# haoningwu3639/StoryGen

Measured on AMD Instinct MI355X. Metric: UNet denoising steps/sec @512x512, 3 prior-frame ctx, bs=1, higher is better.
Workload: dtype f16; 1 GPU; BASELINE configs[1]: StoryGen denoising loop, 512x512 (64x64x4 latent), R=3 prior frames, CFG batch 3, DDIM, SD-1.5 UNet + attn3 (909M params, synthetic fp16 weights); stage=multi-image-condition, samples_per_gpu=1, parallelism=dp1 (one sample per GPU, final all-gather), hipgraph=True, dedup_identical_reference_samples=True, overlap_ref_pass_of_next_step=True, ref_ahead=1, warmup_run=5, split_graphs=False, stream_priority=False, ref_pass_on_cus=0, ref_pass_eager=False, paired_gemm_launches=True, paired_text_image_attention=False, groupnorm_stats_from_epilogues=True, fp16_block_stream=False

## Files before the change

### include/storygen_hip.h

```cpp
#ifndef STORYGEN_HIP_H
#define STORYGEN_HIP_H

#include <stddef.h>
#include <stdint.h>

#ifdef __cplusplus
extern "C" {
#endif

#define SG_OK        0
#define SG_EINVAL   (-1)
#define SG_EUNSUP   (-2)
#define SG_ELAUNCH  (-3)
#define SG_EARCH    (-4)

typedef void* sg_stream_t;
typedef uint16_t sg_half;

int          sg_version(void);
const char*  sg_last_error(void);
int          sg_device_arch(void);
int          sg_device_cus(void);

#define SG_EPI_LINEAR 0
// ... 80 lines not shown
    sg_half*       y;  int64_t ldy;
    int32_t        M, C;
    float          eps;
    int32_t        hidden_split;
} sg_ff_desc;

size_t sg_ff_fused_pack_bytes(int32_t C);
int sg_ff_geglu_fused_f16(const sg_ff_desc* d, sg_stream_t stream);

typedef struct sg_attn_desc {
    const sg_half* q;  int64_t ldq, bsq;
    const sg_half* k;  int64_t ldk, bsk;
    const sg_half* vt; int64_t ldvt, bsvt;
    sg_half*       o;  int64_t ldo, bso;
    int32_t B, H, Nq, Nk, D;
    int32_t kv_batches;
    float   scale;
    const sg_half* k2;  int64_t bsk2;
    const sg_half* vt2; int64_t bsvt2;
    int32_t Nk2, kv2_batches;
} sg_attn_desc;

int sg_attn_fwd_f16(const sg_attn_desc* d, sg_stream_t stream);

int sg_attn_fwd_pair_f16(const sg_attn_desc* d0, const sg_attn_desc* d1, sg_stream_t stream);

enum {
    SG_ATTN_D40_LOOP    = 0,
    SG_ATTN_SHARED_BODY = 1,
    SG_ATTN_GENERAL     = 2,
    SG_ATTN_LEAN        = 3,
    SG_ATTN_KSPLIT      = 4,
    SG_ATTN_LSE         = 5,
    SG_ATTN_F8          = 6
};
typedef struct sg_attn_plan {
    int32_t family, waves, stages, workgroups;
} sg_attn_plan;
typedef struct sg_attn_pair_plan {
    int32_t shared, first;
    sg_attn_plan p0, p1;
    int32_t workgroups;
} sg_attn_pair_plan;
int sg_attn_fwd_plan(const sg_attn_desc* d, int32_t lse, sg_attn_plan* out);
int sg_attn_fwd_pair_plan(const sg_attn_desc* d0, const sg_attn_desc* d1, sg_attn_pair_plan* out);

typedef struct sg_groupnorm_desc {
    const void*    x;  int64_t ldx;
    int32_t        x_f32;
    int32_t        y_pad_w;
    sg_half*       y;  int64_t ldy;
    sg_half*       xcopy; int64_t ldxc;
    const sg_half* gamma; const sg_half* beta;
    int32_t B, HW, C, groups;
    float   eps;
    int32_t silu;
    void*   workspace; size_t workspace_bytes;
    const float* pstats[2];
    int32_t pstats_rows[2], pstats_c0[2], pstats_nc[2];
    const float*   split_ws; int32_t split_count;
    const sg_half* split_bias;
    const float*   split_rowbias; int64_t split_rowbias_ld;
    const void*    split_res; int64_t split_ldr; int32_t split_res_f32;
    void*          split_out; int64_t split_ldo; int32_t split_out_f32;
    int32_t        split_round_f16;
} sg_groupnorm_desc;

// ... 184 lines not shown
```

### storygen_amd/csrc/attention.hip

```cpp
#include "attention_kernel.h"
#include <float.h>

using namespace sgattn;


static int attn_params(const sg_attn_desc* d, AttnParams& p, const char* who) {
    SG_REQUIRE(d != nullptr, "%s: null descriptor", who);
    SG_REQUIRE(d->q && d->k && d->vt && d->o, "%s: null q/k/vt/o", who);
    SG_REQUIRE(d->B > 0 && d->H > 0 && d->Nq > 0 && d->Nk > 0, "%s: bad shape", who);
    if (d->D != 40 && d->D != 80 && d->D != 160)
        return sg_set_error(SG_EUNSUP, "%s: head dim %d not in {40, 80, 160}", who, d->D);
    SG_REQUIRE(d->Nq <= (1 << 30) && d->Nk <= (1 << 30), "%s: Nq and Nk must not exceed 2^30", who);
    SG_REQUIRE(d->scale > 0.f && d->scale <= FLT_MAX, "%s: scale must be finite and > 0", who);
    SG_REQUIRE(d->kv_batches >= 0 && d->kv_batches <= d->B, "%s: kv_batches must be in [0, B]", who);
    SG_REQUIRE(d->kv_batches == 0 || 2 * (int64_t)d->kv_batches >= d->B, "%s: kv_batches must be 0 or at least B / 2", who);
    SG_REQUIRE(d->ldq % 8 == 0 && d->ldk % 8 == 0 && d->ldvt % 8 == 0 && d->ldo % 4 == 0, "%s: row strides", who);
    SG_REQUIRE(d->bsq % 8 == 0 && d->bsk % 8 == 0 && d->bsvt % 8 == 0 && d->bso % 4 == 0, "%s: batch strides", who);
    SG_REQUIRE(sg_aligned16(d->q) && sg_aligned16(d->k) && sg_aligned16(d->vt) && sg_aligned16(d->o), "%s: 16-byte alignment", who);
    const int64_t hd = (int64_t)d->H * d->D;
    SG_REQUIRE(d->ldq >= hd && d->ldk >= hd && d->ldo >= hd, "%s: token stride smaller than H*D", who);
    SG_REQUIRE(d->ldvt >= ((d->Nk + 7) & ~7), "%s: ldvt must cover Nk rounded up to 8 keys", who);
    SG_REQUIRE((int64_t)d->D * d->ldvt < (1ll << 31), "%s: VT head slab too large for 32-bit offsets", who);
    SG_REQUIRE(d->ldk < (1ll << 25), "%s: K tile (64 ldk) too large for 32-bit offsets", who);
    p = AttnParams{};
    p.q = reinterpret_cast<const f16*>(d->q); p.ldq = d->ldq; p.bsq = d->bsq;
    p.k = reinterpret_cast<const f16*>(d->k); p.ldk = d->ldk; p.bsk = d->bsk;
    p.vt = reinterpret_cast<const f16*>(d->vt); p.ldvt = d->ldvt; p.bsvt = d->bsvt;
    p.o = reinterpret_cast<f16*>(d->o); p.ldo = d->ldo; p.bso = d->bso;
    p.B = d->B; p.H = d->H; p.Nq = d->Nq; p.Nk = d->Nk;
    p.kv_batches = d->kv_batches > 0 ? d->kv_batches : d->B;
    p.scale_log2 = d->scale * 1.44269504088896340736f;
    if (d->kv2_batches > 0) {
        SG_REQUIRE(d->k2 && d->vt2 && d->Nk2 > 0 && d->kv2_batches <= p.kv_batches, "%s: kv2_batches needs k2, vt2, Nk2 and at most kv_batches rows", who);
        SG_REQUIRE(d->bsk2 % 8 == 0 && d->bsvt2 % 8 == 0 && sg_aligned16(d->k2) && sg_aligned16(d->vt2), "%s: k2 / vt2 strides and alignment", who);
        SG_REQUIRE(d->ldvt >= ((d->Nk2 + 7) & ~7), "%s: ldvt must cover Nk2 rounded up to 8 keys", who);
        p.k2 = reinterpret_cast<const f16*>(d->k2); p.bsk2 = d->bsk2;
        p.vt2 = reinterpret_cast<const f16*>(d->vt2); p.bsvt2 = d->bsvt2;
        p.Nk2 = d->Nk2; p.kv2 = d->kv2_batches;
    }
    return SG_OK;
}


static bool attn_big(const sg_attn_desc* d) { return (long)sg_cdiv(d->Nq, 128) * d->H * d->B >= 512; }

static int attn_plan_grid(sg_attn_plan& pl, const sg_attn_desc* d, int family, int waves, int stages, const char* who) {
    const int64_t wgs = (int64_t)sg_cdiv(d->Nq, family == SG_ATTN_KSPLIT ? 32 : 32 * waves) * d->H * d->B;
    SG_REQUIRE(wgs < (1ll << 31), "%s: %lld workgroups do not fit a grid", who, (long long)wgs);
    pl.family = family; pl.waves = waves; pl.stages = stages; pl.workgroups = (int32_t)wgs;
    return SG_OK;
}

static int attn_plan(const sg_attn_desc* d, bool lse, sg_attn_plan& pl, const char* who) {
    if (lse) return attn_plan_grid(pl, d, SG_ATTN_LSE, 4, 3, who);
    const bool big = attn_big(d);
    const SgOptions& opt = sg_options();
    if (d->D == 40) {
        if (big && opt.attn_d40_general) return attn_plan_grid(pl, d, SG_ATTN_GENERAL, 4, 3, who);
        if (big && opt.attn_lean) return attn_plan_grid(pl, d, SG_ATTN_LEAN, 4, 3, who);
        return attn_plan_grid(pl, d, opt.attn_d40_loop == 1 ? SG_ATTN_SHARED_BODY : SG_ATTN_D40_LOOP, big ? 4 : 2, big ? 3 : 2, who);
    }
    if (d->D == 160 && opt.attn_d160 == 4 && d->Nq <= 256 && d->Nk > KVBLK && (long)sg_cdiv(d->Nq, 32) * d->H * d->B <= 256)
        return attn_plan_grid(pl, d, SG_ATTN_KSPLIT, 4, 1, who);
    return attn_plan_grid(pl, d, SG_ATTN_GENERAL, 4, 3, who);
}

static int attn_launch(const AttnParams& p, int D, const sg_attn_plan& pl, hipStream_t st) {
    const bool big = pl.waves == 4;
    switch (pl.family) {
    case SG_ATTN_LSE:
        if (D == 40) launch_attn<40, 4, 3, true, false, true>(p, st);
        else if (D == 80) launch_attn<80, 4, 3, true>(p, st);
        else launch_attn<160, 4, 3, true>(p, st);
        return SG_OK;
    case SG_ATTN_D40_LOOP: big ? launch_attn_d40<4, 3>(p, st) : launch_attn_d40<2, 2>(p, st); return SG_OK;
    case SG_ATTN_SHARED_BODY: big ? launch_attn<40, 4, 3>(p, st) : launch_attn<40, 2, 2>(p, st); return SG_OK;
    case SG_ATTN_LEAN: launch_attn<40, 4, 3, false, true>(p, st); return SG_OK;
    case SG_ATTN_KSPLIT: launch_attn_ksplit<160, 4>(p, st); return SG_OK;
    case SG_ATTN_GENERAL:
        if (D == 40) launch_attn<40, 4, 3, false, false, true>(p, st);
        else if (D == 80) launch_attn<80, 4, 3>(p, st);
        else launch_attn<160, 4, 3>(p, st);
        return SG_OK;
    }
    return sg_set_error(SG_EINVAL, "attention: internal: no kernel for plan family %d", pl.family);
}

static int attn_fwd(const sg_attn_desc* d, float* lse2, sg_stream_t stream) {
    const char* who = lse2 ? "sg_attn_fwd_lse_f16" : "sg_attn_fwd_f16";
    AttnParams p;
    sg_attn_plan pl;
    if (int rc = attn_params(d, p, "sg_attn_fwd_f16")) return rc;
    if (int rc = attn_plan(d, lse2 != nullptr, pl, "sg_attn_fwd_f16")) return rc;
    p.lse2 = lse2;
    if (int rc = attn_launch(p, d->D, pl, (hipStream_t)stream)) return rc;
    SG_CHECK_LAUNCH(who);
    return SG_OK;
}

extern "C" int sg_attn_fwd_f16(const sg_attn_desc* d, sg_stream_t stream) { return attn_fwd(d, nullptr, stream); }

extern "C" int sg_attn_fwd_plan(const sg_attn_desc* d, int32_t lse, sg_attn_plan* out) {
    SG_REQUIRE(out != nullptr, "sg_attn_fwd_plan: null plan");
    AttnParams p;
    if (int rc = attn_params(d, p, "sg_attn_fwd_plan")) return rc;
    return attn_plan(d, lse != 0, *out, "sg_attn_fwd_plan");
}

static int attn_pair_plan(const sg_attn_desc* d0, const sg_attn_desc* d1, sg_attn_pair_plan& pr, const char* who) {
    const SgOptions& opt = sg_options();
    const bool same = d0->D == d1->D && d0->B == d1->B && d0->H == d1->H && d0->Nq == d1->Nq;
// ... 55 lines not shown
```

### storygen_amd/csrc/attention_kernel.h

```cpp
#pragma once
#include "common.h"
#include <stdlib.h>
#include <type_traits>

namespace sgattn {


constexpr int KVBLK = 64;
constexpr float RESCALE_THR = 6.0f;

struct AttnParams {
    const f16* q; long ldq, bsq;
    const f16* k; long ldk, bsk;
    const f16* vt; long ldvt, bsvt;
    f16* o; long ldo, bso;
    int B, H, Nq, Nk, kv_batches, nqb;
    const f16* k2; long bsk2; const f16* vt2; long bsvt2; int Nk2, kv2;
    float scale_log2;
    float* lse2;
};

__device__ __forceinline__ void glds16(const f16* g, char* lds_wave_base) {
    __builtin_amdgcn_global_load_lds((const __attribute__((address_space(1))) void*)g,
                                     (__attribute__((address_space(3))) void*)lds_wave_base, 16, 0, 0);
}
template <int N>
__device__ __forceinline__ void wait_vmcnt() {
    asm volatile("s_waitcnt vmcnt(%0)" ::"n"(N) : "memory");
}

template <int D>
__device__ __forceinline__ int kswz(int row) {
    return D == 40 ? 0 : (D == 80 ? ((row >> 3) & 1) : ((row >> 2) & 3));
}

constexpr int F40_KPAD = 2688;
constexpr int F40_ONES = 128;

template <int D, int NIMG>
constexpr int attn_smem_bytes() {
    return D == 40 ? F40_KPAD + NIMG * (KVBLK * D * 2 + D * 128 + F40_ONES) : NIMG * (KVBLK * D * 2 + D * 128) + (D % 16 == 0 ? 0 : 16);
}

template <int D, int NW, int S, bool LSE, bool LEAN = false, bool GENERAL = false, bool KSPLIT = false>
__device__ __forceinline__ void attn_fwd_body(const AttnParams& p, char* smem, const int block, const int nblocks) {
    constexpr int SUB = KSPLIT ? NW : 1;
    constexpr bool F40 = D == 40 && !GENERAL;
    constexpr int DC = D / 8;
    constexpr int NDK = (D + 15) / 16;
    constexpr int DT = (D + 31) / 32;
    constexpr int KROW = D * 2;
    constexpr int K_BYTES = KVBLK * KROW;
    constexpr int V_BYTES = D * 128;
    constexpr int K_SEG = K_BYTES / 1024, V_SEG = V_BYTES / 1024, NSEG = K_SEG + V_SEG;
    constexpr int TSTAGE = K_BYTES + V_BYTES + (F40 ? F40_ONES : 0);
    constexpr int STAGE = SUB * TSTAGE;
    constexpr int RING0 = F40 ? F40_KPAD : 0;
    constexpr int MAXL = (NSEG + NW - 1) / NW;
    constexpr int REM = NSEG % NW;
    static_assert(KSPLIT ? (S == 1 && !LSE && !(D == 40 && !GENERAL)) : (S == 2 || S == 3), "2 or 3 stages; key split: one stage of NW tiles");
    static_assert(!KSPLIT || NW * (8 + DT * 64) * 64 <= S * SUB * (KVBLK * D * 2 + D * 128), "the merge images of the waves fit the dead ring");
    static_assert((S - 1) * MAXL < 64, "vmcnt is a 6-bit counter");
    static_assert(RING0 + S * STAGE + (F40 || D % 16 == 0 ? 0 : 16) <= attn_smem_bytes<D, S * SUB>(), "LDS size");
    static_assert(!F40 || (32 * KROW + 16 <= F40_KPAD && F40_KPAD % 128 == 0), "K pad constants of both 32-key blocks");

    const int t = threadIdx.x, lane = t & 63, l31 = lane & 31, hi = lane >> 5;
    const int wave = __builtin_amdgcn_readfirstlane(t >> 6);
    const int work = xcd_remap(block, nblocks);
    const int bh = work / p.nqb, qb = work - bh * p.nqb;
    const int h = bh / p.B, b = bh - h * p.B;
    const int kvb = b < p.kv_batches ? b : b - (p.B - p.kv_batches);
    const bool short_row = kvb < p.kv2;
    const int Nk = short_row ? p.Nk2 : p.Nk;
    const int q0 = KSPLIT ? qb * 32 : (qb * NW + wave) * 32;
    const f16* Q = p.q + (long)b * p.bsq + (long)h * D;
    const f16* K = (short_row ? p.k2 + (long)kvb * p.bsk2 : p.k + (long)(kvb - p.kv2) * p.bsk) + (long)h * D;
    const f16* VT = (short_row ? p.vt2 + (long)kvb * p.bsvt2 : p.vt + (long)(kvb - p.kv2) * p.bsvt) + (long)h * D * p.ldvt;
    const int nkp8 = (Nk + 7) & ~7;

    if constexpr (F40) {
        if (t < 8) {
            const unsigned v = (t & 3) == 0 ? 0x3C003C00u : 0u;
            *reinterpret_cast<unsigned*>(smem + ((t >> 2) ? 32 * KROW : 0) + 4 * (t & 3)) = v;
        }
        for (int i = t; i < S * SUB * (F40_ONES / 4); i += 64 * NW) {
            const int img = i / (F40_ONES / 4), w = i - img * (F40_ONES / 4);
            *reinterpret_cast<unsigned*>(smem + RING0 + img * TSTAGE + K_BYTES + V_BYTES + 4 * w) = 0x3C003C00u;
        }
        asm volatile("s_waitcnt lgkmcnt(0)" ::: "memory");
    }

    auto coords = [&](int g, int& row, int& col) __attribute__((always_inline)) {
        row = col = 0;
        if (g < K_SEG) {
            const int s = g * 64 + lane;
            const int kl = s / DC, cs = s - kl * DC;
            row = kl;
            col = (cs ^ kswz<D>(kl)) * 8;
        } else if (g < NSEG) {
            const int s = (g - K_SEG) * 64 + lane;
            const int d = s >> 3, cs = s & 7;
            row = d * (int)p.ldvt;
            col = (cs ^ ((d >> 1) & 7)) * 8;
        }
    };
    unsigned off[MAXL];
#pragma unroll
    for (int i = 0; i < MAXL; ++i) {
        const int g = i * NW + wave;
        int row, col;
        coords(g, row, col);
        off[i] = g < K_SEG ? (unsigned)(row * (int)p.ldk + col) : (unsigned)(row + col);
    }
    const int ntiles = (Nk + KVBLK - 1) / KVBLK;
    auto issue_tile = [&](int tile, char* base) __attribute__((always_inline)) {
        const int key0 = tile * KVBLK;
        if (key0 + KVBLK <= Nk) {
            const f16* Kt = K + (long)key0 * p.ldk;
            const f16* Vt = VT + key0;
#pragma unroll
            for (int i = 0; i < MAXL; ++i) {
                const int g = i * NW + wave;
                const f16* src = (g < K_SEG ? Kt : Vt) + off[i];
                if ((i + 1) * NW <= NSEG || g < NSEG) glds16(src, base + g * 1024);
            }
        } else {
#pragma unroll
            for (int i = 0; i < MAXL; ++i) {
                const int g = i * NW + wave;
                int row, col;
                coords(g, row, col);
                if (g < K_SEG) {
                    const int key = min(key0 + row, Nk - 1);
                    glds16(K + (long)key * p.ldk + col, base + g * 1024);
                } else if (g < NSEG) {
                    const int kc = min(key0 + col, nkp8 - 8);
                    glds16(VT + row + kc, base + g * 1024);
                }
            }
        }
    };
    auto issue = [&](int group, int stage) __attribute__((always_inline)) {
#pragma unroll
        for (int sub = 0; sub < SUB; ++sub)
            if (group * SUB + sub < ntiles) issue_tile(group * SUB + sub, smem + RING0 + stage * STAGE + sub * TSTAGE);
    };

    f16x8 qf[NDK];
    {
        const int qi = min(q0 + l31, p.Nq - 1);
#pragma unroll
        for (int s = 0; s < NDK; ++s) {
            const int d0 = s * 16 + hi * 8;
            H8 x; x.u = make_uint4(0, 0, 0, 0);
            if (d0 < D) x.u = ldg16(Q + (long)qi * p.ldq + d0);
            if constexpr (F40) {
#pragma unroll
                for (int j = 0; j < 8; ++j) x.h[j] = (f16)((float)x.h[j] * p.scale_log2);
            }
            qf[s] = x.v;
        }
    }
    __builtin_amdgcn_s_waitcnt(0x0F70);

    f32x16 oacc[DT];
#pragma unroll
    for (int i = 0; i < DT; ++i)
#pragma unroll
        for (int r = 0; r < 16; ++r) oacc[i][r] = 0.f;
    float m_run = F40 ? 0.f : -INFINITY;
    float l_run = 0.f;

    const int ngroups = (ntiles + SUB - 1) / SUB;
#pragma unroll
    for (int s = 0; s < S - 1; ++s)
        if (s < ngroups) issue(s, s);

    const int prow = (l31 & ~12) | ((l31 & 4) << 1) | ((l31 & 8) >> 1);
    constexpr bool UNR = D == 40;
    int rt_stage = 0;
    for (int group0 = 0; group0 < ngroups; group0 += (UNR ? S : 1)) {
#pragma unroll
    for (int ustage = 0; ustage < (UNR ? S : 1); ++ustage) {
        const int group = group0 + ustage;
        const int stage = UNR ? ustage : rt_stage;
        if (group < ngroups) {
        if constexpr (KSPLIT) {
            if (group > 0) __builtin_amdgcn_s_barrier();
            issue(group, 0);
            wait_vmcnt<0>();
            __builtin_amdgcn_s_barrier();
        } else {
        if (S == 3 && group + 1 < ngroups) {
            if (REM == 0 || wave < REM) wait_vmcnt<MAXL>();
            else wait_vmcnt<(MAXL > 1 ? MAXL - 1 : 0)>();
        } else {
            wait_vmcnt<0>();
        }
        __builtin_amdgcn_s_barrier();
        if (group + S - 1 < ngroups) {
            int st = stage + S - 1;
            if (st >= S) st -= S;
            issue(group + S - 1, st);
        }
        }
#pragma unroll
      for (int subi = 0; subi < 1; ++subi) {
        const int sub = KSPLIT ? wave : subi;
        const int tile = group * SUB + sub;
        if (tile < ntiles) {
        const char* sK = smem + RING0 + stage * STAGE + sub * TSTAGE;
        const char* sV = sK + K_BYTES;

        f32x16 s[2];
        const f32x16 zero16 = {0.f, 0.f, 0.f, 0.f, 0.f, 0.f, 0.f, 0.f, 0.f, 0.f, 0.f, 0.f, 0.f, 0.f, 0.f, 0.f};
        constexpr bool KBATCH = NDK <= 5;
        if constexpr (KBATCH) {
            f16x8 kf[2][NDK];
            if constexpr (F40) {
                const char* k01 = sK + prow * KROW + hi * 16;
                const char* k2 = hi ? smem : sK + prow * KROW + 64;
#pragma unroll
                for (int kb = 0; kb < 2; ++kb) {
                    kf[kb][0] = *reinterpret_cast<const f16x8*>(k01 + kb * 32 * KROW);
                    kf[kb][1] = *reinterpret_cast<const f16x8*>(k01 + kb * 32 * KROW + 32);
                    kf[kb][2] = *reinterpret_cast<const f16x8*>(k2 + kb * 32 * KROW);
                }
            } else {
#pragma unroll
                for (int kb = 0; kb < 2; ++kb) {
                    const int row = kb * 32 + prow;
                    const char* krow = sK + row * KROW;
                    const int sw = kswz<D>(row);
#pragma unroll
                    for (int st = 0; st < NDK; ++st)
                        kf[kb][st] = *reinterpret_cast<const f16x8*>(krow + (((st * 2 + hi) ^ sw) << 4));
                }
            }
            __builtin_amdgcn_sched_barrier(0);
#pragma unroll
            for (int kb = 0; kb < 2; ++kb)
#pragma unroll
                for (int st = 0; st < NDK; ++st)
                    s[kb] = __builtin_amdgcn_mfma_f32_32x32x16_f16(kf[kb][st], qf[st], st == 0 ? zero16 : s[kb], 0, 0, 0);
        } else {
            const char* krow0 = sK + prow * KROW;
            const char* krow1 = sK + (32 + prow) * KROW;
            const int sw0 = kswz<D>(prow), sw1 = kswz<D>(32 + prow);
            f16x8 k0 = *reinterpret_cast<const f16x8*>(krow0 + ((hi ^ sw0) << 4));
            f16x8 k1 = *reinterpret_cast<const f16x8*>(krow1 + ((hi ^ sw1) << 4));
#pragma unroll
            for (int st = 0; st < NDK; ++st) {
                f16x8 k0n = k0, k1n = k1;
                if (st + 1 < NDK) {
                    k0n = *reinterpret_cast<const f16x8*>(krow0 + ((((st + 1) * 2 + hi) ^ sw0) << 4));
                    k1n = *reinterpret_cast<const f16x8*>(krow1 + ((((st + 1) * 2 + hi) ^ sw1) << 4));
                }
                __builtin_amdgcn_sched_barrier(0);
                s[0] = __builtin_amdgcn_mfma_f32_32x32x16_f16(k0, qf[st], st == 0 ? zero16 : s[0], 0, 0, 0);
                s[1] = __builtin_amdgcn_mfma_f32_32x32x16_f16(k1, qf[st], st == 0 ? zero16 : s[1], 0, 0, 0);
                k0 = k0n; k1 = k1n;
            }
        }
        constexpr bool VPRE = DT <= 3 && !LEAN;
        constexpr int DLAST = F40 ? D : D - 1;
        f16x8 vf[VPRE ? 4 : 1][DT];
        if constexpr (VPRE) {
#pragma unroll
            for (int ks = 0; ks < 4; ++ks)
#pragma unroll
                for (int i = 0; i < DT; ++i) {
                    const int d = min(i * 32 + l31, DLAST);
                    vf[ks][i] = *reinterpret_cast<const f16x8*>(sV + d * 128 + (((ks * 2 + hi) ^ ((d >> 1) & 7)) << 4));
                }
        }
        if ((tile + 1) * KVBLK > Nk) {
#pragma unroll
            for (int kb = 0; kb < 2; ++kb)
#pragma unroll
                for (int r = 0; r < 16; ++r) {
                    const int key = tile * KVBLK + kb * 32 + 16 * (r >> 3) + 8 * hi + (r & 7);
                    if (key >= Nk) s[kb][r] = -INFINITY;
                }
        }
        float mx = s[0][0];
#pragma unroll
        for (int kb = 0; kb < 2; ++kb)
#pragma unroll
            for (int r = 0; r < 16; ++r) mx = fmaxf(mx, s[kb][r]);
        if constexpr (F40) {
            mx = fmaxf(mx, __shfl_xor(mx, 32, 64));
            if (tile == 0 || __builtin_amdgcn_ballot_w64(mx > RESCALE_THR) != 0) {
                float m_new = m_run + (tile == 0 ? mx : fmaxf(mx, 0.f));
                m_new = fminf(fmaxf(m_new, -60000.f), 60000.f);
                const f16 mh = (f16)m_new;
                const f16 ml = (f16)(m_new - (float)mh);
                m_new = (float)mh + (float)ml;
                const float delta = m_new - m_run;
                if (tile != 0) {
                    const float alpha = __builtin_amdgcn_exp2f(-delta);
#pragma unroll
                    for (int i = 0; i < DT; ++i)
#pragma unroll
                        for (int r = 0; r < 16; ++r) oacc[i][r] *= alpha;
                }
#pragma unroll
                for (int kb = 0; kb < 2; ++kb)
#pragma unroll
                    for (int r = 0; r < 16; ++r) s[kb][r] -= delta;
                m_run = m_new;
                if (hi) { qf[NDK - 1][0] = -mh; qf[NDK - 1][1] = -ml; }
            }
#pragma unroll
            for (int kb = 0; kb < 2; ++kb)
// ... 64 lines not shown
    }

    float l_tot;
    if constexpr (F40) l_tot = oacc[DT - 1][4];
    else l_tot = l_run + __shfl_xor(l_run, 32, 64);
    if constexpr (KSPLIT) {
        constexpr int IMG = (8 + DT * 64) * 64;
        __builtin_amdgcn_s_barrier();
        if (wave > 0) {
            float* img = reinterpret_cast<float*>(smem + (wave - 1) * IMG);
            img[lane] = m_run;
            img[64 + lane] = l_tot;
#pragma unroll
            for (int i = 0; i < DT; ++i)
#pragma unroll
                for (int r = 0; r < 16; ++r) img[128 + (i * 16 + r) * 64 + lane] = oacc[i][r];
        }
        asm volatile("s_waitcnt lgkmcnt(0)" ::: "memory");
        __builtin_amdgcn_s_barrier();
        if (wave > 0) return;
#pragma unroll
        for (int w = 1; w < NW; ++w) {
            const float* img = reinterpret_cast<const float*>(smem + (w - 1) * IMG);
            const float m_o = img[lane], l_o = img[64 + lane];
            const float m_new = fmaxf(m_run, m_o);
            const float fa = __builtin_amdgcn_exp2f(m_run - m_new), fb = __builtin_amdgcn_exp2f(m_o - m_new);
            l_tot = l_tot * fa + l_o * fb;
            m_run = m_new;
#pragma unroll
            for (int i = 0; i < DT; ++i)
#pragma unroll
                for (int r = 0; r < 16; ++r) oacc[i][r] = oacc[i][r] * fa + img[128 + (i * 16 + r) * 64 + lane] * fb;
        }
    }
    const float inv = 1.0f / l_tot;
    const int qi = q0 + l31;
    if constexpr (LSE) {
        if (hi == 0 && qi < p.Nq) p.lse2[((long)b * p.H + h) * p.Nq + qi] = m_run + __log2f(l_tot);
    }
    if (qi < p.Nq) {
        f16* O = p.o + (long)b * p.bso + (long)qi * p.ldo + (long)h * D;
#pragma unroll
        for (int i = 0; i < DT; ++i)
#pragma unroll
            for (int g = 0; g < 4; ++g) {
                const int d0 = i * 32 + 8 * g + 4 * hi;
                if (d0 < D) {
                    f16x4 w = {(f16)(oacc[i][4 * g + 0] * inv), (f16)(oacc[i][4 * g + 1] * inv),
                               (f16)(oacc[i][4 * g + 2] * inv), (f16)(oacc[i][4 * g + 3] * inv)};
                    *reinterpret_cast<f16x4*>(O + d0) = w;
                }
            }
    }
}

template <int NW, int S>
__device__ __forceinline__ void attn_d40_body(const AttnParams& p, char* smem, const int block, const int nblocks) {
    constexpr int D = 40, DC = D / 8, NDK = 3, DT = 2, KROW = D * 2;
    constexpr int K_BYTES = KVBLK * KROW, V_BYTES = D * 128;
    constexpr int K_SEG = K_BYTES / 1024, V_SEG = V_BYTES / 1024;
    constexpr int TSTAGE = K_BYTES + V_BYTES + F40_ONES, RING0 = F40_KPAD;
    constexpr int NPAIR = (K_SEG - 1) / NW;
    static_assert((NW == 2 || NW == 4) && (S == 2 || S == 3), "2 or 4 waves, 2 or 3 stages");
    static_assert(K_SEG == 5 && V_SEG == 5 && NPAIR * NW == 4, "4 segments of K and of V^T over the waves + one of each for waves 0 and 1");
    static_assert(RING0 + S * TSTAGE <= attn_smem_bytes<D, S>(), "LDS size");

// ... 268 lines not shown
__global__ __launch_bounds__(64 * NW) __attribute__((amdgpu_waves_per_eu(3))) void attn_d40_kernel(const AttnParams p) {
    __shared__ __attribute__((aligned(16))) char smem[attn_smem_bytes<40, S>()];
    attn_d40_body<NW, S>(p, smem, (int)blockIdx.x, (int)gridDim.x);
}

template <int NW, int S>
__global__ __launch_bounds__(64 * NW) __attribute__((amdgpu_waves_per_eu(3))) void attn_d40_pair_kernel(const AttnParams a, const AttnParams b, const int na) {
    __shared__ __attribute__((aligned(16))) char smem[attn_smem_bytes<40, S>()];
    if ((int)blockIdx.x < na) attn_d40_body<NW, S>(a, smem, (int)blockIdx.x, na);
    else attn_d40_body<NW, S>(b, smem, (int)blockIdx.x - na, (int)gridDim.x - na);
}

template <int NW, int S>
void launch_attn_d40(const AttnParams& p0, hipStream_t st) {
    AttnParams p = p0;
    p.nqb = sg_cdiv(p.Nq, 32 * NW);
    hipLaunchKernelGGL((attn_d40_kernel<NW, S>), dim3(p.nqb * p.H * p.B), dim3(64 * NW), 0, st, p);
}

template <int NW, int S>
void launch_attn_d40_pair(const AttnParams& a0, const AttnParams& b0, hipStream_t st) {
    AttnParams a = a0, b = b0;
    a.nqb = sg_cdiv(a.Nq, 32 * NW); b.nqb = sg_cdiv(b.Nq, 32 * NW);
    const int na = a.nqb * a.H * a.B, nb = b.nqb * b.H * b.B;
    hipLaunchKernelGGL((attn_d40_pair_kernel<NW, S>), dim3(na + nb), dim3(64 * NW), 0, st, a, b, na);
}

template <int D, int NW, int S, bool LSE = false, bool LEAN = false, bool GENERAL = false>
__global__ __launch_bounds__(64 * NW) void attn_fwd_kernel(const AttnParams p) {
    __shared__ __attribute__((aligned(16))) char smem[attn_smem_bytes<D, S>()];
    attn_fwd_body<D, NW, S, LSE, LEAN, GENERAL>(p, smem, (int)blockIdx.x, (int)gridDim.x);
}

template <int D, int NW>
__global__ __launch_bounds__(64 * NW) void attn_fwd_ksplit_kernel(const AttnParams p) {
    __shared__ __attribute__((aligned(16))) char smem[attn_smem_bytes<D, NW>()];
    attn_fwd_body<D, NW, 1, false, false, false, true>(p, smem, (int)blockIdx.x, (int)gridDim.x);
}

template <int D, int NW>
void launch_attn_ksplit(const AttnParams& p0, hipStream_t st) {
    AttnParams p = p0;
    p.nqb = sg_cdiv(p.Nq, 32);
    hipLaunchKernelGGL((attn_fwd_ksplit_kernel<D, NW>), dim3(p.nqb * p.H * p.B), dim3(64 * NW), 0, st, p);
}

template <int D, int NW, int S>
__global__ __launch_bounds__(64 * NW) void attn_fwd_pair_kernel(const AttnParams a, const AttnParams b, const int na) {
    __shared__ __attribute__((aligned(16))) char smem[attn_smem_bytes<D, S>()];
    if ((int)blockIdx.x < na) attn_fwd_body<D, NW, S, false>(a, smem, (int)blockIdx.x, na);
    else attn_fwd_body<D, NW, S, false>(b, smem, (int)blockIdx.x - na, (int)gridDim.x - na);
}

template <int D, int NW, int S, bool LSE = false, bool LEAN = false, bool GENERAL = false>
void launch_attn(const AttnParams& p0, hipStream_t st) {
    AttnParams p = p0;
    p.nqb = sg_cdiv(p.Nq, 32 * NW);
    hipLaunchKernelGGL((attn_fwd_kernel<D, NW, S, LSE, LEAN, GENERAL>), dim3(p.nqb * p.H * p.B), dim3(64 * NW), 0, st, p);
}

template <int D, int NW, int S>
void launch_attn_pair(const AttnParams& a0, const AttnParams& b0, hipStream_t st) {
    AttnParams a = a0, b = b0;
    a.nqb = sg_cdiv(a.Nq, 32 * NW); b.nqb = sg_cdiv(b.Nq, 32 * NW);
    const int na = a.nqb * a.H * a.B, nb = b.nqb * b.H * b.B;
    hipLaunchKernelGGL((attn_fwd_pair_kernel<D, NW, S>), dim3(na + nb), dim3(64 * NW), 0, st, a, b, na);
// ... 5 lines not shown
```

### storygen_amd/csrc/common.h

```cpp
#pragma once
#include <hip/hip_runtime.h>
#include <stdint.h>
#include <stdio.h>
#include <stdarg.h>

#include "../../include/storygen_hip.h"

typedef _Float16 f16;
typedef f16 f16x2 __attribute__((ext_vector_type(2)));
typedef f16 f16x4 __attribute__((ext_vector_type(4)));
typedef f16 f16x8 __attribute__((ext_vector_type(8)));
typedef float f32x4 __attribute__((ext_vector_type(4)));
typedef float f32x16 __attribute__((ext_vector_type(16)));

int sg_set_error(int code, const char* fmt, ...);

#define SG_REQUIRE(cond, ...)                                   \
    do {                                                        \
        if (!(cond)) return sg_set_error(SG_EINVAL, __VA_ARGS__); \
    } while (0)

#define SG_CHECK_LAUNCH(name)                                                                  \
    do {                                                                                       \
        hipError_t e__ = hipGetLastError();                                                    \
        if (e__ != hipSuccess) return sg_set_error(SG_ELAUNCH, "%s: %s", name, hipGetErrorString(e__)); \
    } while (0)

static inline bool sg_aligned16(const void* p) { return (reinterpret_cast<uintptr_t>(p) & 15u) == 0; }
static inline int sg_cdiv(long a, long b) { return (int)((a + b - 1) / b); }

struct SgOptions {
    int tile_m = 0, tile_n = 0;
    int no_pipe = 0, no_split = 0;
    int no_nmajor = 0;
    int pipe_stages = 3;
    int lat_tiles = 640;
    int lat_min_kt = 8, lat_max_kt = 64;
    int lat_stages = 4;
    int lat_mask = 62;
    int big_m = 0, big_bm = 0, big_bn = 0;
    int fat_m = 0;
    int lat_wide = 0, lat_wide_m = 256;
    int attn_d160 = 4;
    int attn_lean = 0;
    int attn_d40_general = 0;
    int attn_d40_loop = 0;
    int gn_no_fused = 0, gn_wide = 1;
    int gn_fused_nt = 1024;
    int gn_chunks = 0;
    int ff_variant = 3;
    long gn_fused_max = -1;
};
SgOptions& sg_options();

__device__ __forceinline__ uint4 ldg16(const void* p) { return *reinterpret_cast<const uint4*>(p); }
__device__ __forceinline__ void stg16(void* p, uint4 v) { *reinterpret_cast<uint4*>(p) = v; }

union H8 {
    uint4 u;
    f16x8 v;
    f16 h[8];
};

__device__ __forceinline__ void load8f(const void* base, long off, bool f32, float (&v)[8]) {
    if (f32) {
        const float* q = reinterpret_cast<const float*>(base) + off;
        const float4 a = *reinterpret_cast<const float4*>(q), b = *reinterpret_cast<const float4*>(q + 4);
        v[0] = a.x; v[1] = a.y; v[2] = a.z; v[3] = a.w; v[4] = b.x; v[5] = b.y; v[6] = b.z; v[7] = b.w;
    } else {
        H8 h; h.u = ldg16(reinterpret_cast<const f16*>(base) + off);
#pragma unroll
        for (int j = 0; j < 8; ++j) v[j] = (float)h.h[j];
    }
}
__device__ __forceinline__ void store8h(f16* p, const float (&v)[8]) {
    H8 o;
// ... 32 lines not shown
```

### storygen_amd/csrc/misc.hip

```cpp
#include "common.h"
#include <string.h>

static thread_local char g_err[512] = "";

SgOptions& sg_options() {
    static SgOptions o;
    return o;
}

extern "C" int sg_debug_set_option(const char* name, int64_t value) {
    if (!name) return sg_set_error(SG_EINVAL, "sg_debug_set_option: null name");
    SgOptions& o = sg_options();
    struct Entry { const char* n; int* p; };
    const Entry table[] = {{"tile_m", &o.tile_m}, {"tile_n", &o.tile_n}, {"no_pipe", &o.no_pipe}, {"no_split", &o.no_split},
                           {"no_nmajor", &o.no_nmajor}, {"attn_d160", &o.attn_d160}, {"gn_no_fused", &o.gn_no_fused},
                           {"gn_wide", &o.gn_wide}, {"attn_lean", &o.attn_lean}, {"attn_d40_general", &o.attn_d40_general}, {"attn_d40_loop", &o.attn_d40_loop},
                           {"gn_fused_nt", &o.gn_fused_nt}, {"pipe_stages", &o.pipe_stages}, {"ff_variant", &o.ff_variant},
                           {"gn_chunks", &o.gn_chunks}, {"lat_tiles", &o.lat_tiles}, {"lat_min_kt", &o.lat_min_kt},
                           {"lat_max_kt", &o.lat_max_kt}, {"lat_stages", &o.lat_stages}, {"lat_wide", &o.lat_wide}, {"lat_mask", &o.lat_mask}, {"lat_wide_m", &o.lat_wide_m}, {"fat_m", &o.fat_m}, {"big_m", &o.big_m}, {"big_bm", &o.big_bm}, {"big_bn", &o.big_bn}};
    for (const Entry& e : table)
        if (strcmp(e.n, name) == 0) {
            if (e.p == &o.attn_d160 && value != 3 && value != 4)
                return sg_set_error(SG_EINVAL, "sg_debug_set_option: attn_d160 must be 3 (query split) or 4 (key split where it applies)");
            *e.p = (int)value;
            return SG_OK;
        }
    if (strcmp(name, "gn_fused_max") == 0) {
        o.gn_fused_max = (long)value;
        return SG_OK;
    }
    if (strcmp(name, "reset") == 0) {
        o = SgOptions{};
        return SG_OK;
    }
    return sg_set_error(SG_EINVAL, "sg_debug_set_option: unknown option '%s'", name);
}

int sg_set_error(int code, const char* fmt, ...) {
    va_list ap;
    va_start(ap, fmt);
    vsnprintf(g_err, sizeof(g_err), fmt, ap);
    va_end(ap);
    return code;
}

extern "C" int sg_version(void) { return 1; }
extern "C" const char* sg_last_error(void) { return g_err; }

extern "C" int sg_device_arch(void) {
    int dev = 0;
    hipDeviceProp_t prop;
    if (hipGetDevice(&dev) != hipSuccess || hipGetDeviceProperties(&prop, dev) != hipSuccess)
        return sg_set_error(SG_ELAUNCH, "sg_device_arch: no HIP device");
    const char* name = prop.gcnArchName;
    if (strncmp(name, "gfx", 3) != 0) return sg_set_error(SG_EARCH, "sg_device_arch: unexpected arch '%s'", name);
    return (int)strtol(name + 3, nullptr, 10);
// ... 413 lines not shown
```

### storygen_amd/ops.py

```python
from __future__ import annotations

import ctypes as C
from typing import Optional

import torch

from . import _lib
from ._lib import AttnDesc, AttnPairPlan, AttnPlan, ConvDesc, FfDesc, GemmDesc, GnPlan, GroupNormDesc, check

lib = _lib.load()

EPI_LINEAR = 0
EPI_GEGLU = 1
F_OUT_F32, F_RES1_F32, F_RES2_F32 = 1, 2, 4

TILE_TABLE = {}
TUNE_SINK = None


def _apply_tile(d, tile, split_k, sig, mn):
    if tile is not None:
        d.tile_m, d.tile_n = tile[0], tile[1]
        if len(tile) > 2:
            d.tile_waves = tile[2]
# ... 433 lines not shown
    keys = [Nk] * B
    if short is not None:
        k2, vt2 = short
        _f16(k2, "k2"), _f16(vt2, "vt2")
        n2, Nk2 = k2.shape[0], k2.shape[1]
        if (k2.dim() != 3 or vt2.dim() != 3 or k2.shape[2] != Cq or tuple(vt2.shape[:2]) != (n2, Cq) or vt2.shape[2] < ((Nk2 + 7) & ~7)
                or k2.stride(-1) != 1 or vt2.stride(-1) != 1 or k2.stride(1) != k.stride(1) or vt2.stride(1) != vt.stride(1)):
            raise ValueError("attention: short rows must be [n, Nk2, H*D] / [n, H*D, Nk2] views with the token / row strides of k / vt")
        d.k2, d.bsk2, d.vt2, d.bsvt2 = k2.data_ptr(), k2.stride(0), vt2.data_ptr(), vt2.stride(0)
        d.Nk2, d.kv2_batches = Nk2, n2
        d.kv_batches = Bk = Bk + n2
        keys = [Nk2 if (b if b < Bk else b - (B - Bk)) < n2 else Nk for b in range(B)]
    if d.kv_batches > B:
        raise ValueError(f"attention: {d.kv_batches} K/V rows for {B} query batches")
    shape = f"B{B} H{heads} Nq{Nq} Nk{Nk}" + (f" ({d.kv2_batches}x Nk{d.Nk2})" if short is not None else "")
    return d, 4.0 * heads * Nq * D * float(sum(keys)), shape


def attention(q: torch.Tensor, k: torch.Tensor, vt: torch.Tensor, out: torch.Tensor, heads: int, scale: float,
              nk: Optional[int] = None, short: Optional[tuple] = None) -> torch.Tensor:
    d, flops, shape = _attn_fwd_desc(q, k, vt, out, heads, scale, nk, short)
    with _timed(f"attention_d{d.D}", flops, shape):
        check(lib.sg_attn_fwd_f16(C.byref(d), _stream()), "sg_attn_fwd_f16")
    return out


def attention_pair(a: tuple, b: tuple, heads: int, scale: float) -> None:
    da, fa, sa = _attn_fwd_desc(*a[:4], heads, scale, *a[4:])
    db, fb, sb = _attn_fwd_desc(*b[:4], heads, scale, *b[4:])
    with _timed(f"attention_d{da.D}", fa + fb, f"{sa} + {sb}"):
        check(lib.sg_attn_fwd_pair_f16(C.byref(da), C.byref(db), _stream()), "sg_attn_fwd_pair_f16")


ATTN_FAMILIES = ("d40_loop", "shared_body", "general", "lean", "ksplit", "lse", "f8")


def _attn_plan_tuple(pl) -> tuple:
    return (ATTN_FAMILIES[pl.family], pl.waves, pl.stages, pl.workgroups)


def attention_plan(q: torch.Tensor, k: torch.Tensor, vt: torch.Tensor, out: torch.Tensor, heads: int, scale: float,
                   nk: Optional[int] = None, short: Optional[tuple] = None, lse: bool = False) -> tuple:
    d, _, _ = _attn_fwd_desc(q, k, vt, out, heads, scale, nk, short)
    pl = AttnPlan()
    check(lib.sg_attn_fwd_plan(C.byref(d), int(lse), C.byref(pl)), "sg_attn_fwd_plan")
    return _attn_plan_tuple(pl)


def attention_pair_plan(a: tuple, b: tuple, heads: int, scale: float) -> tuple:
    da, _, _ = _attn_fwd_desc(*a[:4], heads, scale, *a[4:])
    db, _, _ = _attn_fwd_desc(*b[:4], heads, scale, *b[4:])
    pr = AttnPairPlan()
    check(lib.sg_attn_fwd_pair_plan(C.byref(da), C.byref(db), C.byref(pr)), "sg_attn_fwd_pair_plan")
    return (bool(pr.shared), pr.first, _attn_plan_tuple(pr.p0), _attn_plan_tuple(pr.p1), pr.workgroups)


def attention_f8_plan(B: int, heads: int, Nq: int) -> tuple:
    pl = AttnPlan()
    check(lib.sg_attn_fwd_f8_plan(B, heads, Nq, C.byref(pl)), "sg_attn_fwd_f8_plan")
    return _attn_plan_tuple(pl)


def attention_f8_bytes(B: int, heads: int, N: int, transposed: bool) -> int:
    return lib.sg_attn_f8_bytes(B, heads, N, int(transposed))


def attention_f8(q: torch.Tensor, k: torch.Tensor, vt: torch.Tensor, out: torch.Tensor, heads: int, scale: float,
# ... 623 lines not shown
                     dq: torch.Tensor, heads: int, scale: float) -> torch.Tensor:
    d = _attn_bwd_desc(q, k, v, dout, ld2, heads, scale)
    _f16(kt, "kt"), _f16(dq, "dq")
    d.kt, d.ldkt, d.bskt = kt.data_ptr(), kt.stride(1), kt.stride(0)
    d.dq, d.lddq, d.bsdq = dq.data_ptr(), dq.stride(1), dq.stride(0)
    with _timed("attention_bwd", 6.0 * d.B * d.H * d.Nq * d.Nk * d.D, f"dq B{d.B} H{d.H} Nq{d.Nq} Nk{d.Nk} D{d.D}"):
        check(lib.sg_attn_bwd_dq_f16(C.byref(d), _stream()), "sg_attn_bwd_dq_f16")
    return dq


def attention_bwd_dkv(q: torch.Tensor, qt: torch.Tensor, k: torch.Tensor, v: torch.Tensor, dout: torch.Tensor, dot: torch.Tensor,
                      ld2: torch.Tensor, dkt: torch.Tensor, dvt: torch.Tensor, heads: int, scale: float):
    d = _attn_bwd_desc(q, k, v, dout, ld2, heads, scale)
    for n, t in (("qt", qt), ("dot", dot), ("dkt", dkt), ("dvt", dvt)):
        _f16(t, n)
    d.qt, d.ldqt, d.bsqt = qt.data_ptr(), qt.stride(1), qt.stride(0)
    d.dot, d.lddot, d.bsdot = dot.data_ptr(), dot.stride(1), dot.stride(0)
    d.dkt, d.lddkt, d.bsdkt = dkt.data_ptr(), dkt.stride(1), dkt.stride(0)
    d.dvt, d.lddvt, d.bsdvt = dvt.data_ptr(), dvt.stride(1), dvt.stride(0)
    with _timed("attention_bwd", 8.0 * d.B * d.H * d.Nq * d.Nk * d.D, f"dkv B{d.B} H{d.H} Nq{d.Nq} Nk{d.Nk} D{d.D}"):
        check(lib.sg_attn_bwd_dkv_f16(C.byref(d), _stream()), "sg_attn_bwd_dkv_f16")
    return dkt, dvt


def debug_set_tile(bm: int = 0, bn: int = 0, no_pipe: bool = False) -> None:
    check(lib.sg_debug_set_tile(bm, bn, int(no_pipe)), "sg_debug_set_tile")


def debug_set_option(name: str, value: int) -> None:
    check(lib.sg_debug_set_option(name.encode(), int(value)), "sg_debug_set_option")


_ENV_OPTIONS = {"SG_NO_NMAJOR": "no_nmajor", "SG_NO_PIPE": "no_pipe", "SG_NO_SPLIT": "no_split",
                "SG_ATTN_D160": "attn_d160",
                "SG_FF_VARIANT": "ff_variant", "SG_PIPE_STAGES": "pipe_stages", "SG_GN_FUSED_NT": "gn_fused_nt", "SG_GN_CHUNKS": "gn_chunks", "SG_ATTN_LEAN": "attn_lean", "SG_ATTN_D40_GENERAL": "attn_d40_general", "SG_ATTN_D40_LOOP": "attn_d40_loop","SG_NO_GN_FUSED": "gn_no_fused", "SG_GN_WIDE": "gn_wide", "SG_GN_FUSED_MAX": "gn_fused_max",
                "SG_LAT_TILES": "lat_tiles", "SG_LAT_MIN_KT": "lat_min_kt", "SG_LAT_MAX_KT": "lat_max_kt", "SG_LAT_STAGES": "lat_stages", "SG_LAT_WIDE": "lat_wide", "SG_LAT_MASK": "lat_mask", "SG_LAT_WIDE_M": "lat_wide_m", "SG_FAT_M": "fat_m", "SG_BIG_M": "big_m", "SG_BIG_BM": "big_bm", "SG_BIG_BN": "big_bn"}


def apply_env_options() -> dict:
    import os
    done = {}
    for var, name in _ENV_OPTIONS.items():
        if os.environ.get(var, "") != "":
            debug_set_option(name, int(os.environ[var]))
            done[name] = int(os.environ[var])
    if os.environ.get("SG_TILE"):
        bm, bn = (int(v) for v in os.environ["SG_TILE"].split(","))
        debug_set_option("tile_m", bm), debug_set_option("tile_n", bn)
        done["tile"] = (bm, bn)
    return done


def debug_mfma_f8(a_bytes: torch.Tensor, b_bytes: torch.Tensor, scale_a: int = 127, scale_b: int = 127) -> torch.Tensor:
    if a_bytes.dtype != torch.uint8 or tuple(a_bytes.shape) != (64, 32) or not a_bytes.is_cuda or not a_bytes.is_contiguous():
        raise TypeError("debug_mfma_f8: a must be a contiguous CUDA uint8 [64, 32]")
    if b_bytes.dtype != torch.uint8 or tuple(b_bytes.shape) != (64, 32) or not b_bytes.is_cuda or not b_bytes.is_contiguous():
        raise TypeError("debug_mfma_f8: b must be a contiguous CUDA uint8 [64, 32]")
    out = torch.empty(64, 16, dtype=torch.float32, device=a_bytes.device)
    check(lib.sg_debug_mfma_f8_32x32x64(a_bytes.data_ptr(), b_bytes.data_ptr(), out.data_ptr(), scale_a, scale_b, _stream()),
          "sg_debug_mfma_f8_32x32x64")
    return out


def debug_mfma(a: torch.Tensor, b: torch.Tensor) -> torch.Tensor:
    out = torch.empty(64, 16, dtype=torch.float32, device=a.device)
    check(lib.sg_debug_mfma_32x32x16(a.data_ptr(), b.data_ptr(), out.data_ptr(), _stream()), "sg_debug_mfma_32x32x16")
    return out
# ... 1 lines not shown
```

Before: 80.15 denoising steps/s.

## Split D=80 attention keys into two halves across eight waves and merge

Adds a 'halves' attention family for head dim 80 with small grids and long key sequences. Each workgroup runs two groups of four waves, each on its own half of the key tiles with its own 3-stage LDS ring. The second half writes its running max, sum and partial output to LDS so the first half can merge them. The aim is more parallelism when there are too few query blocks to fill the CUs. In exchange it doubles LDS per workgroup and adds a merge barrier, which may reduce occupancy.

```diff
diff --git a/include/storygen_hip.h b/include/storygen_hip.h
--- a/include/storygen_hip.h
+++ b/include/storygen_hip.h
@@ -136,7 +136,8 @@
     SG_ATTN_LEAN        = 3,
     SG_ATTN_KSPLIT      = 4,
     SG_ATTN_LSE         = 5,
-    SG_ATTN_F8          = 6
+    SG_ATTN_F8          = 6,
+    SG_ATTN_HALVES      = 7
 };
 typedef struct sg_attn_plan {
     int32_t family, waves, stages, workgroups;
diff --git a/storygen_amd/csrc/attention.hip b/storygen_amd/csrc/attention.hip
--- a/storygen_amd/csrc/attention.hip
+++ b/storygen_amd/csrc/attention.hip
@@ -45,7 +45,8 @@
 static bool attn_big(const sg_attn_desc* d) { return (long)sg_cdiv(d->Nq, 128) * d->H * d->B >= 512; }
 
 static int attn_plan_grid(sg_attn_plan& pl, const sg_attn_desc* d, int family, int waves, int stages, const char* who) {
-    const int64_t wgs = (int64_t)sg_cdiv(d->Nq, family == SG_ATTN_KSPLIT ? 32 : 32 * waves) * d->H * d->B;
+    const int wq = family == SG_ATTN_KSPLIT ? 32 : family == SG_ATTN_HALVES ? 16 * waves : 32 * waves;
+    const int64_t wgs = (int64_t)sg_cdiv(d->Nq, wq) * d->H * d->B;
     SG_REQUIRE(wgs < (1ll << 31), "%s: %lld workgroups do not fit a grid", who, (long long)wgs);
     pl.family = family; pl.waves = waves; pl.stages = stages; pl.workgroups = (int32_t)wgs;
     return SG_OK;
@@ -62,6 +63,11 @@
     }
     if (d->D == 160 && opt.attn_d160 == 4 && d->Nq <= 256 && d->Nk > KVBLK && (long)sg_cdiv(d->Nq, 32) * d->H * d->B <= 256)
         return attn_plan_grid(pl, d, SG_ATTN_KSPLIT, 4, 1, who);
+    if (d->D == 80 && opt.attn_d80 == 8 && (long)sg_cdiv(d->Nq, 128) * d->H * d->B <= 256) {
+        const int shortest = d->kv2_batches > 0 && d->Nk2 < d->Nk ? d->Nk2 : d->Nk;
+        if (sg_cdiv(shortest, KVBLK) >= opt.attn_d80_min_tiles)
+            return attn_plan_grid(pl, d, SG_ATTN_HALVES, 8, 3, who);
+    }
     return attn_plan_grid(pl, d, SG_ATTN_GENERAL, 4, 3, who);
 }
 
@@ -77,6 +83,7 @@
     case SG_ATTN_SHARED_BODY: big ? launch_attn<40, 4, 3>(p, st) : launch_attn<40, 2, 2>(p, st); return SG_OK;
     case SG_ATTN_LEAN: launch_attn<40, 4, 3, false, true>(p, st); return SG_OK;
     case SG_ATTN_KSPLIT: launch_attn_ksplit<160, 4>(p, st); return SG_OK;
+    case SG_ATTN_HALVES: launch_attn_halves<80, 4, 3>(p, st); return SG_OK;
     case SG_ATTN_GENERAL:
         if (D == 40) launch_attn<40, 4, 3, false, false, true>(p, st);
         else if (D == 80) launch_attn<80, 4, 3>(p, st);
diff --git a/storygen_amd/csrc/attention_kernel.h b/storygen_amd/csrc/attention_kernel.h
--- a/storygen_amd/csrc/attention_kernel.h
+++ b/storygen_amd/csrc/attention_kernel.h
@@ -42,7 +42,7 @@
     return D == 40 ? F40_KPAD + NIMG * (KVBLK * D * 2 + D * 128 + F40_ONES) : NIMG * (KVBLK * D * 2 + D * 128) + (D % 16 == 0 ? 0 : 16);
 }
 
-template <int D, int NW, int S, bool LSE, bool LEAN = false, bool GENERAL = false, bool KSPLIT = false>
+template <int D, int NW, int S, bool LSE, bool LEAN = false, bool GENERAL = false, bool KSPLIT = false, bool HALVES = false>
 __device__ __forceinline__ void attn_fwd_body(const AttnParams& p, char* smem, const int block, const int nblocks) {
     constexpr int SUB = KSPLIT ? NW : 1;
     constexpr bool F40 = D == 40 && !GENERAL;
@@ -60,12 +60,15 @@
     constexpr int REM = NSEG % NW;
     static_assert(KSPLIT ? (S == 1 && !LSE && !(D == 40 && !GENERAL)) : (S == 2 || S == 3), "2 or 3 stages; key split: one stage of NW tiles");
     static_assert(!KSPLIT || NW * (8 + DT * 64) * 64 <= S * SUB * (KVBLK * D * 2 + D * 128), "the merge images of the waves fit the dead ring");
+    static_assert(!HALVES || (S == 3 && D == 80 && !KSPLIT && !LSE && !LEAN), "key halves: the D = 80 inference forward on two 3-stage rings");
     static_assert((S - 1) * MAXL < 64, "vmcnt is a 6-bit counter");
     static_assert(RING0 + S * STAGE + (F40 || D % 16 == 0 ? 0 : 16) <= attn_smem_bytes<D, S * SUB>(), "LDS size");
     static_assert(!F40 || (32 * KROW + 16 <= F40_KPAD && F40_KPAD % 128 == 0), "K pad constants of both 32-key blocks");
 
     const int t = threadIdx.x, lane = t & 63, l31 = lane & 31, hi = lane >> 5;
-    const int wave = __builtin_amdgcn_readfirstlane(t >> 6);
+    const int wave = __builtin_amdgcn_readfirstlane(HALVES ? (t >> 6) % NW : t >> 6);
+    const int half = HALVES ? __builtin_amdgcn_readfirstlane(t >> 6) / NW : 0;
+    const int hring = HALVES ? half * (S * STAGE) : 0;
     const int work = xcd_remap(block, nblocks);
     const int bh = work / p.nqb, qb = work - bh * p.nqb;
     const int h = bh / p.B, b = bh - h * p.B;
@@ -112,9 +115,12 @@
         coords(g, row, col);
         off[i] = g < K_SEG ? (unsigned)(row * (int)p.ldk + col) : (unsigned)(row + col);
     }
-    const int ntiles = (Nk + KVBLK - 1) / KVBLK;
+    const int tiles_row = (Nk + KVBLK - 1) / KVBLK;
+    const int tiles_h0 = HALVES ? (tiles_row > 1 ? tiles_row / 2 : 1) : tiles_row;
+    const int tile0 = HALVES && half ? tiles_h0 : 0;
+    const int ntiles = HALVES && half ? tiles_row - tiles_h0 : tiles_h0;
     auto issue_tile = [&](int tile, char* base) __attribute__((always_inline)) {
-        const int key0 = tile * KVBLK;
+        const int key0 = (tile0 + tile) * KVBLK;
         if (key0 + KVBLK <= Nk) {
             const f16* Kt = K + (long)key0 * p.ldk;
             const f16* Vt = VT + key0;
@@ -143,7 +149,7 @@
     auto issue = [&](int group, int stage) __attribute__((always_inline)) {
 #pragma unroll
         for (int sub = 0; sub < SUB; ++sub)
-            if (group * SUB + sub < ntiles) issue_tile(group * SUB + sub, smem + RING0 + stage * STAGE + sub * TSTAGE);
+            if (group * SUB + sub < ntiles) issue_tile(group * SUB + sub, smem + RING0 + hring + stage * STAGE + sub * TSTAGE);
     };
 
     f16x8 qf[NDK];
@@ -172,6 +178,7 @@
     float l_run = 0.f;
 
     const int ngroups = (ntiles + SUB - 1) / SUB;
+    const int ntrips = HALVES ? max(tiles_h0, tiles_row - tiles_h0) : ngroups;
 #pragma unroll
     for (int s = 0; s < S - 1; ++s)
         if (s < ngroups) issue(s, s);
@@ -179,12 +186,12 @@
     const int prow = (l31 & ~12) | ((l31 & 4) << 1) | ((l31 & 8) >> 1);
     constexpr bool UNR = D == 40;
     int rt_stage = 0;
-    for (int group0 = 0; group0 < ngroups; group0 += (UNR ? S : 1)) {
+    for (int group0 = 0; group0 < ntrips; group0 += (UNR ? S : 1)) {
 #pragma unroll
     for (int ustage = 0; ustage < (UNR ? S : 1); ++ustage) {
         const int group = group0 + ustage;
         const int stage = UNR ? ustage : rt_stage;
-        if (group < ngroups) {
+        if (HALVES || group < ngroups) {
         if constexpr (KSPLIT) {
             if (group > 0) __builtin_amdgcn_s_barrier();
             issue(group, 0);
@@ -209,7 +216,7 @@
         const int sub = KSPLIT ? wave : subi;
         const int tile = group * SUB + sub;
         if (tile < ntiles) {
-        const char* sK = smem + RING0 + stage * STAGE + sub * TSTAGE;
+        const char* sK = smem + RING0 + hring + stage * STAGE + sub * TSTAGE;
         const char* sV = sK + K_BYTES;
 
         f32x16 s[2];
@@ -274,12 +281,12 @@
                     vf[ks][i] = *reinterpret_cast<const f16x8*>(sV + d * 128 + (((ks * 2 + hi) ^ ((d >> 1) & 7)) << 4));
                 }
         }
-        if ((tile + 1) * KVBLK > Nk) {
+        if ((tile0 + tile + 1) * KVBLK > Nk) {
 #pragma unroll
             for (int kb = 0; kb < 2; ++kb)
 #pragma unroll
                 for (int r = 0; r < 16; ++r) {
-                    const int key = tile * KVBLK + kb * 32 + 16 * (r >> 3) + 8 * hi + (r & 7);
+                    const int key = (tile0 + tile) * KVBLK + kb * 32 + 16 * (r >> 3) + 8 * hi + (r & 7);
                     if (key >= Nk) s[kb][r] = -INFINITY;
                 }
         }
@@ -410,6 +417,30 @@
 #pragma unroll
                 for (int r = 0; r < 16; ++r) oacc[i][r] = oacc[i][r] * fa + img[128 + (i * 16 + r) * 64 + lane] * fb;
         }
+    }
+    if constexpr (HALVES) {
+        constexpr int DV = D / 2;
+        static_assert(D % 32 == 16 && 2 * DV * 256 <= STAGE, "two O^T images (DV x 64 lanes fp32) per dead stage");
+        float* ml = reinterpret_cast<float*>(smem + 2 * S * STAGE) + wave * 128;
+        int dead = rt_stage + (wave >> 1);
+        if (dead >= S) dead -= S;
+        float* img = reinterpret_cast<float*>(smem + S * STAGE + dead * STAGE + (wave & 1) * (DV * 256));
+        if (half) {
+            ml[lane] = m_run;
+            ml[64 + lane] = l_tot;
+#pragma unroll
+            for (int j = 0; j < DV; ++j) img[j * 64 + lane] = oacc[j >> 4][j & 15];
+        }
+        asm volatile("s_waitcnt lgkmcnt(0)" ::: "memory");
+        __builtin_amdgcn_s_barrier();
+        if (half) return;
+        const float m_o = ml[lane], l_o = ml[64 + lane];
+        const float m_new = fmaxf(m_run, m_o);
+        const float fa = __builtin_amdgcn_exp2f(m_run - m_new), fb = __builtin_amdgcn_exp2f(m_o - m_new);
+        l_tot = l_tot * fa + l_o * fb;
+        m_run = m_new;
+#pragma unroll
+        for (int j = 0; j < DV; ++j) oacc[j >> 4][j & 15] = oacc[j >> 4][j & 15] * fa + img[j * 64 + lane] * fb;
     }
     const float inv = 1.0f / l_tot;
     const int qi = q0 + l31;
@@ -744,6 +775,22 @@
     attn_fwd_body<D, NW, S, LSE, LEAN, GENERAL>(p, smem, (int)blockIdx.x, (int)gridDim.x);
 }
 
+template <int D, int NW, int S>
+constexpr int attn_halves_smem_bytes() { return 2 * attn_smem_bytes<D, S>() + NW * 512; }
+
+template <int D, int NW, int S>
+__global__ __launch_bounds__(128 * NW) void attn_fwd_halves_kernel(const AttnParams p) {
+    __shared__ __attribute__((aligned(16))) char smem[attn_halves_smem_bytes<D, NW, S>()];
+    attn_fwd_body<D, NW, S, false, false, false, false, true>(p, smem, (int)blockIdx.x, (int)gridDim.x);
+}
+
+template <int D, int NW, int S>
+void launch_attn_halves(const AttnParams& p0, hipStream_t st) {
+    AttnParams p = p0;
+    p.nqb = sg_cdiv(p.Nq, 32 * NW);
+    hipLaunchKernelGGL((attn_fwd_halves_kernel<D, NW, S>), dim3(p.nqb * p.H * p.B), dim3(128 * NW), 0, st, p);
+}
+
 template <int D, int NW>
 __global__ __launch_bounds__(64 * NW) void attn_fwd_ksplit_kernel(const AttnParams p) {
     __shared__ __attribute__((aligned(16))) char smem[attn_smem_bytes<D, NW>()];
diff --git a/storygen_amd/csrc/common.h b/storygen_amd/csrc/common.h
--- a/storygen_amd/csrc/common.h
+++ b/storygen_amd/csrc/common.h
@@ -42,6 +42,8 @@
     int fat_m = 0;
     int lat_wide = 0, lat_wide_m = 256;
     int attn_d160 = 4;
+    int attn_d80 = 8;
+    int attn_d80_min_tiles = 16;
     int attn_lean = 0;
     int attn_d40_general = 0;
     int attn_d40_loop = 0;
diff --git a/storygen_amd/csrc/misc.hip b/storygen_amd/csrc/misc.hip
--- a/storygen_amd/csrc/misc.hip
+++ b/storygen_amd/csrc/misc.hip
@@ -13,7 +13,7 @@
     SgOptions& o = sg_options();
     struct Entry { const char* n; int* p; };
     const Entry table[] = {{"tile_m", &o.tile_m}, {"tile_n", &o.tile_n}, {"no_pipe", &o.no_pipe}, {"no_split", &o.no_split},
-                           {"no_nmajor", &o.no_nmajor}, {"attn_d160", &o.attn_d160}, {"gn_no_fused", &o.gn_no_fused},
+                           {"no_nmajor", &o.no_nmajor}, {"attn_d160", &o.attn_d160}, {"attn_d80", &o.attn_d80}, {"attn_d80_min_tiles", &o.attn_d80_min_tiles}, {"gn_no_fused", &o.gn_no_fused},
                            {"gn_wide", &o.gn_wide}, {"attn_lean", &o.attn_lean}, {"attn_d40_general", &o.attn_d40_general}, {"attn_d40_loop", &o.attn_d40_loop},
                            {"gn_fused_nt", &o.gn_fused_nt}, {"pipe_stages", &o.pipe_stages}, {"ff_variant", &o.ff_variant},
                            {"gn_chunks", &o.gn_chunks}, {"lat_tiles", &o.lat_tiles}, {"lat_min_kt", &o.lat_min_kt},
@@ -22,6 +22,10 @@
         if (strcmp(e.n, name) == 0) {
             if (e.p == &o.attn_d160 && value != 3 && value != 4)
                 return sg_set_error(SG_EINVAL, "sg_debug_set_option: attn_d160 must be 3 (query split) or 4 (key split where it applies)");
+            if (e.p == &o.attn_d80 && value != 4 && value != 8)
+                return sg_set_error(SG_EINVAL, "sg_debug_set_option: attn_d80 must be 4 (four waves) or 8 (key halves where they apply)");
+            if (e.p == &o.attn_d80_min_tiles && (value < 1 || value > (1 << 24)))
+                return sg_set_error(SG_EINVAL, "sg_debug_set_option: attn_d80_min_tiles must be in [1, 2^24]");
             *e.p = (int)value;
             return SG_OK;
         }
diff --git a/storygen_amd/ops.py b/storygen_amd/ops.py
--- a/storygen_amd/ops.py
+++ b/storygen_amd/ops.py
@@ -489,7 +489,7 @@
         check(lib.sg_attn_fwd_pair_f16(C.byref(da), C.byref(db), _stream()), "sg_attn_fwd_pair_f16")
 
 
-ATTN_FAMILIES = ("d40_loop", "shared_body", "general", "lean", "ksplit", "lse", "f8")
+ATTN_FAMILIES = ("d40_loop", "shared_body", "general", "lean", "ksplit", "lse", "f8", "halves")
 
 
 def _attn_plan_tuple(pl) -> tuple:
@@ -1179,7 +1179,7 @@
 
 
 _ENV_OPTIONS = {"SG_NO_NMAJOR": "no_nmajor", "SG_NO_PIPE": "no_pipe", "SG_NO_SPLIT": "no_split",
-                "SG_ATTN_D160": "attn_d160",
+                "SG_ATTN_D160": "attn_d160", "SG_ATTN_D80": "attn_d80", "SG_ATTN_D80_MIN_TILES": "attn_d80_min_tiles",
                 "SG_FF_VARIANT": "ff_variant", "SG_PIPE_STAGES": "pipe_stages", "SG_GN_FUSED_NT": "gn_fused_nt", "SG_GN_CHUNKS": "gn_chunks", "SG_ATTN_LEAN": "attn_lean", "SG_ATTN_D40_GENERAL": "attn_d40_general", "SG_ATTN_D40_LOOP": "attn_d40_loop","SG_NO_GN_FUSED": "gn_no_fused", "SG_GN_WIDE": "gn_wide", "SG_GN_FUSED_MAX": "gn_fused_max",
                 "SG_LAT_TILES": "lat_tiles", "SG_LAT_MIN_KT": "lat_min_kt", "SG_LAT_MAX_KT": "lat_max_kt", "SG_LAT_STAGES": "lat_stages", "SG_LAT_WIDE": "lat_wide", "SG_LAT_MASK": "lat_mask", "SG_LAT_WIDE_M": "lat_wide_m", "SG_FAT_M": "fat_m", "SG_BIG_M": "big_m", "SG_BIG_BM": "big_bm", "SG_BIG_BN": "big_bn"}
 
```

Measured after the change: 80.07 denoising steps/s. Within noise of the previous version (-0.1%).
